# lwy2020/MicroMix

Measured on AMD Instinct MI355X. Metric: mixed-MX GEMM TFLOPS (Llama-3-8B 4096x4096x4096, all-MXFP8 activations, MXFP4 weights), higher is better.
Workload: dtype mxfp8 x mxfp4 -> f32 acc -> bf16; 1 GPU; BASELINE.json configs[1]: 4096^3 mixed-MX GEMM, (p4,p6,p8)=(0,0,4096), w4 weights; M=4096, N=4096, K=4096, parallelism=single GPU

## Files before the change

micromix_amd/csrc/mx_gemm_tile.inc:

```
#define MM_SMALL (MM_WM <= 2)
namespace MM_NS {

__device__ __forceinline__ int mm_tid() { return (int)threadIdx.x; }
constexpr int WM = MM_WM, TM = MM_TM, TN = MM_TN;
constexpr int BM = WM * TM * 32, BN = 2 * TN * 32, NT = WM * 2 * 64;
constexpr bool SMALL = MM_SMALL;
constexpr int NTHREADS = SMALL ? 2 * NT : NT;
constexpr int NACC = 16 * TM * TN;
typedef float v16f_t __attribute__((ext_vector_type(16)));
typedef int v8i_t __attribute__((ext_vector_type(8)));
typedef int v4i_sel __attribute__((ext_vector_type(4)));
struct Acc {
#if MM_SMALL
    v16f_t t[TM * TN];
#endif
};
constexpr int X_TILE = BM * 128;
constexpr int SF_BYTES = 1024;

constexpr int LDS_BUDGET = MM_LDS_BUDGET;

template <int N>
__device__ __forceinline__ void wait_vmcnt() {
#if !(MM_DBG & 2048)
    MM_DEVICE_ONLY(asm volatile("s_waitcnt vmcnt(%0)" ::"n"(N) : "memory");)
#endif
}
__device__ __forceinline__ void barrier_lds_only() {
#if (MM_DBG & 1024)
    MM_DEVICE_ONLY(asm volatile("s_waitcnt lgkmcnt(0)" ::: "memory");)
#else
    MM_DEVICE_ONLY(asm volatile("s_waitcnt lgkmcnt(0)\n\ts_barrier" ::: "memory");)
#endif
}

template <int EL, int KD> struct Op;
template <> struct Op<EL_FP8, 128> { static constexpr int PITCH = 128, G128 = 128; };
template <> struct Op<EL_FP6, 128> { static constexpr int PITCH = 128, G128 = 96; };
template <> struct Op<EL_FP4, 128> { static constexpr int PITCH = 64, G128 = 64; };
template <> struct Op<EL_FP4, 256> { static constexpr int PITCH = 128, G128 = 64; };

template <int EL> struct Frag;
template <> struct Frag<EL_FP8> { typedef int type __attribute__((ext_vector_type(8))); };
template <> struct Frag<EL_FP6> { typedef int type __attribute__((ext_vector_type(6))); };
template <> struct Frag<EL_FP4> { typedef int type __attribute__((ext_vector_type(4))); };

template <int EL, int KD> struct FragOfs;
template <> struct FragOfs<EL_FP8, 128> {
    int o[2][2];
    __device__ __forceinline__ void init(int row, int kb) {
        const int sw = (row >> 1) & 7, rb = row * 128;
#pragma unroll
        for (int h = 0; h < 2; ++h) {
            o[h][0] = rb + (((4 * h + kb) ^ sw) << 4);
            o[h][1] = rb + (((4 * h + 2 + kb) ^ sw) << 4);
        }
    }
};
template <> struct FragOfs<EL_FP4, 128> {
    int o[2][1];
    __device__ __forceinline__ void init(int row, int kb) {
        const int sw = (row >> 2) & 3, rb = row * 64;
#pragma unroll
        for (int h = 0; h < 2; ++h) o[h][0] = rb + (((2 * h + kb) ^ sw) << 4);
    }
};
template <> struct FragOfs<EL_FP4, 256> {
    int o[4][1];
    __device__ __forceinline__ void init(int row, int kb) {
        const int sw = (row >> 1) & 7, rb = row * 128;
#pragma unroll
        for (int h = 0; h < 4; ++h) o[h][0] = rb + (((2 * h + kb) ^ sw) << 4);
    }
};
template <> struct FragOfs<EL_FP6, 128> {
    int o[2][3];
    __device__ __forceinline__ void init(int row, int kb) {
        const int sw = (row >> 1) & 7, rb = row * 128;
#pragma unroll
        for (int h = 0; h < 2; ++h)
#pragma unroll
            for (int i = 0; i < 3; ++i) {
                const int u = 3 * (2 * h + kb) + i;
// ... 38 lines not shown
    const u4_t hi = *(lds_u4)(unsigned long)a1;
    return typename Frag<EL>::type{(int)lo.x, (int)lo.y, (int)lo.z, (int)lo.w, (int)hi.x, (int)hi.y, (int)hi.z, (int)hi.w};
}
template <class G, int EL> using FragOfsOf = std::conditional_t<G::XEL == EL_FP8 && G::WEL == EL_FP8 && !MM_SMALL, FragOfsC<EL, G::KD>, FragOfs<EL, G::KD>>;

template <int T, int XEL, int WEL, int HSEL, bool FENCE = false>
__device__ __forceinline__ void mfma_tile(const typename Frag<XEL>::type &x, const typename Frag<WEL>::type &w, int sx,
                                          int sw) {
#if !(MM_DBG & 1)
    if constexpr (FENCE) {
        MM_DEVICE_ONLY(asm volatile("s_nop 1\n\tv_mfma_scale_f32_32x32x64_f8f6f4 a[%c7:%c8], %0, %1, a[%c7:%c8], %2, %3 "
                                    "op_sel_hi:[%c4,%c4,0] cbsz:%c5 blgp:%c6"
                                    :
                                    : "v"(x), "v"(w), "v"(sx), "v"(sw), "i"(HSEL), "i"(ElemTraits<XEL>::HW),
                                      "i"(ElemTraits<WEL>::HW), "i"(16 * T), "i"(16 * T + 15)
                                    : MM_ACC, "memory");)
    } else {
        MM_DEVICE_ONLY(asm volatile("s_nop 1\n\tv_mfma_scale_f32_32x32x64_f8f6f4 a[%c7:%c8], %0, %1, a[%c7:%c8], %2, %3 "
                                    "op_sel_hi:[%c4,%c4,0] cbsz:%c5 blgp:%c6"
                                    :
                                    : "v"(x), "v"(w), "v"(sx), "v"(sw), "i"(HSEL), "i"(ElemTraits<XEL>::HW),
                                      "i"(ElemTraits<WEL>::HW), "i"(16 * T), "i"(16 * T + 15)
                                    : MM_ACC);)
    }
#else
    MM_DEVICE_ONLY(asm volatile("" ::"v"(x), "v"(w), "v"(sx), "v"(sw));)
#endif
}

template <int I>
__device__ __forceinline__ float acc_read() {
    float v = 0.0f;
    MM_DEVICE_ONLY(asm volatile("v_accvgpr_read_b32 %0, a[%c1]" : "=v"(v) : "i"(I) : MM_ACC);)
    return v;
}
template <int I>
__device__ __forceinline__ void acc_write(float v) {
    MM_DEVICE_ONLY(asm volatile("v_accvgpr_write_b32 a[%c1], %0" : : "v"(v), "i"(I) : MM_ACC);)
}
__device__ __forceinline__ void acc_settle() { MM_DEVICE_ONLY(asm volatile("s_nop 15\n\ts_nop 7" ::: MM_ACC);) }

template <int I, int N>
struct AccLoop {
    static __device__ __forceinline__ void zero() {
        acc_write<I>(0.0f);
        AccLoop<I + 1, N>::zero();
    }
    static __device__ __forceinline__ void round_bf16() {
        static_assert(I % 8 == 0 && N % 8 == 0, "accumulators are rounded eight at a time");
        MM_DEVICE_ONLY(unsigned r0, r1, r2, r3, r4, r5, r6, r7, p0, p1, p2, p3;
                       asm volatile("v_accvgpr_read_b32 %0, a[%c12]\n\tv_accvgpr_read_b32 %1, a[%c13]\n\t"
                                    "v_accvgpr_read_b32 %2, a[%c14]\n\tv_accvgpr_read_b32 %3, a[%c15]\n\t"
                                    "v_accvgpr_read_b32 %4, a[%c16]\n\tv_accvgpr_read_b32 %5, a[%c17]\n\t"
                                    "v_accvgpr_read_b32 %6, a[%c18]\n\tv_accvgpr_read_b32 %7, a[%c19]\n\t"
                                    "v_cvt_pk_bf16_f32 %8, %0, %1\n\tv_cvt_pk_bf16_f32 %9, %2, %3\n\t"
                                    "v_cvt_pk_bf16_f32 %10, %4, %5\n\tv_cvt_pk_bf16_f32 %11, %6, %7\n\t"
                                    "v_lshlrev_b32 %0, 16, %8\n\tv_and_b32 %1, 0xffff0000, %8\n\t"
                                    "v_lshlrev_b32 %2, 16, %9\n\tv_and_b32 %3, 0xffff0000, %9\n\t"
                                    "v_lshlrev_b32 %4, 16, %10\n\tv_and_b32 %5, 0xffff0000, %10\n\t"
                                    "v_lshlrev_b32 %6, 16, %11\n\tv_and_b32 %7, 0xffff0000, %11\n\t"
                                    "v_accvgpr_write_b32 a[%c12], %0\n\tv_accvgpr_write_b32 a[%c13], %1\n\t"
                                    "v_accvgpr_write_b32 a[%c14], %2\n\tv_accvgpr_write_b32 a[%c15], %3\n\t"
                                    "v_accvgpr_write_b32 a[%c16], %4\n\tv_accvgpr_write_b32 a[%c17], %5\n\t"
                                    "v_accvgpr_write_b32 a[%c18], %6\n\tv_accvgpr_write_b32 a[%c19], %7"
                                    : "=&v"(r0), "=&v"(r1), "=&v"(r2), "=&v"(r3), "=&v"(r4), "=&v"(r5), "=&v"(r6), "=&v"(r7),
                                      "=&v"(p0), "=&v"(p1), "=&v"(p2), "=&v"(p3)
                                    : "i"(I), "i"(I + 1), "i"(I + 2), "i"(I + 3), "i"(I + 4), "i"(I + 5), "i"(I + 6), "i"(I + 7)
                                    : MM_ACC);)
        AccLoop<I + 8, N>::round_bf16();
    }
    static __device__ __forceinline__ void store(float *p) {
        static_assert(I % 4 == 0 && N % 4 == 0, "four accumulator registers per store");
        typedef float v4f __attribute__((ext_vector_type(4)));
        [[maybe_unused]] const v4f v = {acc_read<I>(), acc_read<I + 1>(), acc_read<I + 2>(), acc_read<I + 3>()};
        MM_DEVICE_ONLY(asm volatile("global_store_dwordx4 %0, %1, off sc0 sc1\n\ts_nop 1" ::"v"(p + (I / 4) * NT * 4), "v"(v) : "memory");)
        AccLoop<I + 4, N>::store(p);
    }
};
template <int N>
struct AccLoop<N, N> {
    static __device__ __forceinline__ void zero() {}
    static __device__ __forceinline__ void round_bf16() {}
    static __device__ __forceinline__ void store(float *) {}
};

typedef int rsrc_t __attribute__((ext_vector_type(4)));

__device__ __forceinline__ rsrc_t make_rsrc(const uint8_t *base, unsigned bytes) {
    const unsigned long long v = (unsigned long long)base;
    rsrc_t r;
    r[0] = __builtin_amdgcn_readfirstlane((int)(unsigned)v);
    r[1] = __builtin_amdgcn_readfirstlane((int)((unsigned)(v >> 32) & 0xFFFFu));
    r[2] = __builtin_amdgcn_readfirstlane((int)bytes);
    r[3] = 0x00020000;
    return r;
}

__device__ __forceinline__ void dma16(const rsrc_t &rsrc, int voff, int soff, unsigned lds_addr) {
#if (MM_DBG & 2)
    MM_DEVICE_ONLY(asm volatile("" ::"v"(voff), "s"(rsrc), "s"(lds_addr), "s"(soff));)
    return;
#endif
    MM_DEVICE_ONLY(unsigned keep;
                   asm volatile("s_nop 4\n\ts_mov_b32 %0, m0\n\ts_mov_b32 m0, %3\n\ts_nop 0\n\t"
                                "buffer_load_dwordx4 %1, %2, %4 offen lds\n\ts_mov_b32 m0, %0"
                                : "=&s"(keep)
                                : "v"(voff), "s"(rsrc), "s"(lds_addr), "s"(soff)
                                : "memory");)
}

typedef int v4i_t __attribute__((ext_vector_type(4)));
__device__ __forceinline__ __amdgpu_buffer_rsrc_t make_brsrc(const uint8_t *base, unsigned bytes) {
    const unsigned long long v = (unsigned long long)base;
    const unsigned lo = __builtin_amdgcn_readfirstlane((unsigned)v), hi = __builtin_amdgcn_readfirstlane((unsigned)(v >> 32));
    return __builtin_amdgcn_make_buffer_rsrc((void *)(((unsigned long long)hi << 32) | lo), 0,
                                             (int)__builtin_amdgcn_readfirstlane(bytes), 0x00020000);
}
constexpr int OOB = 1 << 30;

__device__ __forceinline__ unsigned lds_address(const uint8_t *p) {
    return (unsigned)(unsigned long long)p;
}

template <int PITCH, int ROWS>
struct OperandDma {
    static constexpr int CPR = PITCH / 16;
    static constexpr int PIECES = ROWS * CPR / NT;
    static_assert(ROWS * CPR % NT == 0, "tile must be a whole number of wave instructions");
    static constexpr int ROWS_PER_IT = NT / CPR;
    rsrc_t rsrc;
    __amdgpu_buffer_rsrc_t brsrc;
    int voff0;
    int rowbytes;
    int g128;
    __device__ __forceinline__ void init(const uint8_t *base, int row0, int nrows, int nslab128, int g128_) {
        g128 = __builtin_amdgcn_readfirstlane(g128_);
        rowbytes = __builtin_amdgcn_readfirstlane(nslab128 * g128);
        int rows = nrows - row0;
        rows = rows > ROWS ? ROWS : rows;
        if constexpr (SMALL) brsrc = make_brsrc(base + (size_t)row0 * (unsigned)rowbytes, (unsigned)rows * (unsigned)rowbytes);
        if constexpr (!SMALL) rsrc = make_rsrc(base + (size_t)row0 * (unsigned)rowbytes, (unsigned)rows * (unsigned)rowbytes);
        const int tid = mm_tid() & (NT - 1);
        const int row = tid / CPR;
        int c;
        if constexpr (CPR == 4) c = (tid & 3) ^ ((row >> 2) & 3);
        else c = (tid & 7) ^ ((row >> 1) & 7);
        if (g128 == 96) c = c >= 6 ? c - 6 : c;
        voff0 = row * rowbytes + c * 16;
    }
    template <int IT>
    __device__ __forceinline__ void piece(int slab128, const uint8_t *lds_tile, int wave) const {
#if (MM_DBG & 16384)
        if constexpr (CPR == 8 && PIECES == 4) {
            const int tid = mm_tid() & (NT - 1);
            const int v = ((IT >> 1) * (NT / 4) + (tid >> 2)) * rowbytes + ((tid & 3) + 4 * (IT & 1)) * 16;
            dma16(rsrc, v, __builtin_amdgcn_readfirstlane(slab128 * g128),
                  __builtin_amdgcn_readfirstlane(lds_address(lds_tile) + (IT * NT + wave * 64) * 16));
            return;
        }
#endif
        dma16(rsrc, voff0 + IT * ROWS_PER_IT * rowbytes, __builtin_amdgcn_readfirstlane(slab128 * g128),
              __builtin_amdgcn_readfirstlane(lds_address(lds_tile) + (IT * NT + wave * 64) * 16));
    }
    template <int IT>
    __device__ __forceinline__ v4i_t load(int slab128, int oob) const {
        return __builtin_amdgcn_raw_buffer_load_b128(brsrc, voff0 + IT * ROWS_PER_IT * rowbytes + oob,
// ... 514 lines not shown
#pragma unroll
                    for (int e = 0; e < 8; ++e)
                        if (n + e < a.N) dst[e] = (uint16_t)(w[e >> 1] >> (16 * (e & 1)));
                }
            }
        }
    }
    template <int GI, int I = 0>
    __device__ __forceinline__ void mfmas_with_rounding() {
        if constexpr (I < 8) {
            mfma<(GI >> 1), (GI & 1), I>();
            if constexpr (GI > 0) round_chunk<((GI - 1) >> 1), ((GI - 1) & 1), I>();
            mfmas_with_rounding<GI, I + 1>();
        }
    }
    template <int GI>
    __device__ __forceinline__ void group() {
        if constexpr (GI < 4) {
            constexpr int TM_ = GI >> 1, P = GI & 1;
            if constexpr (P == 0) load_x<TM_>();
            load_w<2 * P>(ws[0]);
            load_w<2 * P + 1>(ws[1]);
            mfmas_with_rounding<GI>();
        } else {
#if MM_CLOCKS
            if (a.clock_out != nullptr && mm_tid() == 0) {
                a.clock_out[4 * blockIdx.x] = __builtin_amdgcn_s_memtime();
                a.clock_out[4 * blockIdx.x + 1] = __builtin_amdgcn_s_memrealtime();
            }
#endif
            round_chunk<1, 1, 0>(); round_chunk<1, 1, 1>(); round_chunk<1, 1, 2>(); round_chunk<1, 1, 3>();
            round_chunk<1, 1, 4>(); round_chunk<1, 1, 5>(); round_chunk<1, 1, 6>(); round_chunk<1, 1, 7>();
        }
        if constexpr (GI > 0) store_group<((GI - 1) >> 1), ((GI - 1) & 1)>();
        if constexpr (GI < 4) group<GI + 1>();
    }
};

template <class G, class FX, class FW>
__device__ __forceinline__ void run_tail(const GemmArgs &a, int m0, int n0, uint8_t *smem, int c2, int c1, int cf, const Scales<G::KD> &sca,
                                         const FX &fx, const FW &fw, int gx, int gw) {
    const int lane = mm_tid() & 63, wave = __builtin_amdgcn_readfirstlane(mm_tid() >> 6);
    const int wm = wave >> 1, wn = wave & 1, li = lane & 31, kb = lane >> 5;
    wait_vmcnt<0>();
    barrier_lds_only();
    TailTM<G, FX, FW> t{a, smem + c2 * G::STAGE, smem + c1 * G::STAGE, smem + cf * G::STAGE + wave * (32 * TAIL_EP), fx, fw};
    t.sca = sca;
    load_scales<G>(t.scb, t.sb, gx, gw, li, kb);
    t.m0w = m0 + wm * (TM * 32);
    t.n0w = n0 + wn * (TN * 32);
    t.lane = lane;
    t.li = li;
    t.hi = lane >> 5;
    t.sel = (lane & 1) ? 0x03020706u : 0x05040100u;
#pragma unroll
    for (int tn = 0; tn < TN; ++tn) {
        const int n = t.n0w + tn * 32 + li;
        t.bias[tn] = (a.bias != nullptr && n < a.N) ? bf16_bits_to_f32(a.bias[n]) : 0.0f;
    }
    t.template group<0>();
}


template <class G, bool CH, class NX, class PRE, bool TAIL = false>
__device__ __forceinline__ int run_slabs_big(const GemmArgs &a, int Q, int nslab128, int first128, int count, int m0, int n0,
                                             uint8_t *smem, PRE pre, int pref_in, int cur0, const NX &nxd, int nx_pref) {
    constexpr int XEL = G::XEL, WEL = G::WEL, KD = G::KD;
    constexpr bool SAME = CH && (KD == NX::KD), DIFF = CH && (KD != NX::KD);
    static_assert(!TAIL || G::NSTAGE == 3, "the tail runs on a three-stage ring");
    static_assert(!SAME || (NX::STAGE == G::STAGE && NX::NPIECES == SlabDma<G>::NPIECES), "a same-geometry successor continues the ring");
    const int lane = mm_tid() & 63, wave = __builtin_amdgcn_readfirstlane(mm_tid() >> 6);
    const int wm = wave >> 1, wn = wave & 1;
    const int li = lane & 31, kb = lane >> 5;

    SlabDma<G> dma;
    init_slab_dma<G>(dma, a, Q, m0, n0, nslab128, first128, wave);

    constexpr int NS = G::NSTAGE;
    static_assert(NS == 2 || NS == 3, "this pipeline is written out for two or three stages");
    static_assert(!DIFF || NS == 2, "a successor of another geometry needs the two-stage ring (see Chaining above run_slabs_big)");
    auto stage_at = [&](int i) { return smem + i * G::STAGE; };
    auto next_of = [&](int i) { return (i + 1 == NS) ? 0 : i + 1; };
    int cur = cur0;
    const int vcount = count + (SAME ? nx_pref : 0);
    {
        int st = cur;
#pragma unroll
        for (int v = 0; v < NS; ++v) {
            if (v >= pref_in) {
                if (v < count) dma.all(v, stage_at(st));
                else if (SAME && v < vcount) nxd.all(v - count, stage_at(st));
            }
            st = next_of(st);
        }
    }
    if (pref_in == 0) {
        pre();
        if (NS == 3 && vcount > 2) wait_slabs<2>(dma);
        else if (vcount > 1) wait_slabs<1>(dma);
        else wait_slabs<0>(dma);
        barrier_lds_only();
    }

    FragOfsOf<G, XEL> fx;
    FragOfsOf<G, WEL> fw;
    fx.init(wm * (TM * 32) + li, kb);
    fw.init(wn * (TN * 32) + li, kb);
    typename Frag<XEL>::type x0[TM], x1[TM];
    typename Frag<WEL>::type w0[TN], w1[TN];
    Scales<KD> sc;
#pragma unroll
    for (int t = 0; t < TM; ++t) x0[t] = load_frag<XEL, KD, 0>(stage_at(cur), fx, t);
#pragma unroll
    for (int t = 0; t < TN; ++t) w0[t] = load_frag<WEL, KD, 0>(stage_at(cur) + G::OFF_W, fw, t);
    const int gx = ((m0 & 127) >> 5) + wm * TM, gw = ((n0 & 127) >> 5) + wn * TN;
    load_scales<G>(sc, stage_at(cur), gx, gw, li, kb);
    if (pref_in != 0) pre();

#ifdef MM_PRESSURE
    int keep_[MM_PRESSURE];
#pragma unroll
    for (int i = 0; i < MM_PRESSURE; ++i) { keep_[i] = lane * (i + 3); MM_DEVICE_ONLY(asm volatile("" : "+v"(keep_[i]));) }
#endif
    for (int s = 0; s < (TAIL ? count - 2 : count); ++s) {
        const int nxt = next_of(cur);
        uint8_t *st_cur = stage_at(cur);
        uint8_t *st_nxt = stage_at(nxt);
        inner_steps<G, 0>(x0, x1, w0, w1, sc, fx, fw, st_cur);
        if (NS == 3 && s + 2 < vcount) wait_slabs<1>(dma);
        else wait_slabs<0>(dma);
        barrier_lds_only();
        Scales<KD> scn;
        load_scales<G>(scn, st_nxt, gx, gw, li, kb);
        auto lx = [&](auto t) { x0[decltype(t)::value] = load_frag<XEL, KD, 0>(st_nxt, fx, decltype(t)::value); };
        auto lw = [&](auto t) { w0[decltype(t)::value] = load_frag<WEL, KD, 0>(st_nxt + G::OFF_W, fw, decltype(t)::value); };
        constexpr int HL = G::KSTEPS - 1;
        const int v = s + NS;
        if (v < count) {
            mfma_step<XEL, WEL, (HL & 1), SlabPiecesT<SlabDma<G>>>(x1, w1, sc.x[HL >> 1], sc.w[HL >> 1], SlabPiecesT<SlabDma<G>>{dma, v, st_cur}, lx, lw);
        } else if (SAME && v - count < nx_pref) {
            mfma_step<XEL, WEL, (HL & 1), SlabPiecesT<NX>>(x1, w1, sc.x[HL >> 1], sc.w[HL >> 1], SlabPiecesT<NX>{nxd, v - count, st_cur}, lx, lw);
        } else if (DIFF && nx_pref > 0 && v == count) {
            mfma_step<XEL, WEL, (HL & 1), SlabPiecesT<NX>>(x1, w1, sc.x[HL >> 1], sc.w[HL >> 1], SlabPiecesT<NX>{nxd, 0, smem}, lx, lw);
        } else if (DIFF && nx_pref > 1 && v == count + 1) {
            mfma_step<XEL, WEL, (HL & 1), TwoSlabPieces<NX>>(x1, w1, sc.x[HL >> 1], sc.w[HL >> 1], TwoSlabPieces<NX>{nxd, nx_pref, smem}, lx, lw);
        } else {
            mfma_step<XEL, WEL, (HL & 1), NoDma>(x1, w1, sc.x[HL >> 1], sc.w[HL >> 1], NoDma{}, lx, lw);
        }
        sc = scn;
        cur = nxt;
    }
#ifdef MM_PRESSURE
#pragma unroll
    for (int i = 0; i < MM_PRESSURE; ++i) { MM_DEVICE_ONLY(asm volatile("" ::"v"(keep_[i]));) }
#endif
    if constexpr (TAIL) {
        run_tail<G>(a, m0, n0, smem, cur, next_of(cur), next_of(next_of(cur)), sc, fx, fw, gx, gw);
    }
    return cur;
}

template <class G, bool CH, class NX, class PRE, bool TAIL = false>
__device__ __forceinline__ int run_slabs(Acc &acc, const GemmArgs &a, int Q, int nslab128, int first128, int count, int m0, int n0,
                                         uint8_t *smem, PRE pre, int pref_in, int cur0, const NX &nxd, int nx_pref) {
    if constexpr (SMALL) {
        static_assert(!TAIL, "the tail belongs to the 8-wave pipeline");
        run_slabs_small<G>(acc, a, Q, nslab128, first128, count, m0, n0, smem, pre);
        return 0;
    } else {
        return run_slabs_big<G, CH, NX, PRE, TAIL>(a, Q, nslab128, first128, count, m0, n0, smem, pre, pref_in, cur0, nxd, nx_pref);
    }
}

template <bool W4> struct Segs {
    using N256 = Geom<EL_FP4, EL_FP4, 256>;
    using N128 = Geom<EL_FP4, EL_FP4, 128>;
    using S = Geom<EL_FP6, (W4 ? EL_FP4 : EL_FP6), 128>;
    using O = Geom<EL_FP8, (W4 ? EL_FP4 : EL_FP8), 128>;
    using DmaSO = SlabDma<S>;
    static_assert(std::is_same<SlabDma<S>, SlabDma<O>>::value && S::NSTAGE == O::NSTAGE, "S and O chain through one ring");
    static constexpr bool CHAIN = (MM_CHAIN && W4 && BM == 256 && !SMALL && MM_FP4_KD256 && N256::NSTAGE == 2 && S::STAGE <= N256::STAGE &&
                                   S::NSTAGE * S::STAGE <= LDS_BUDGET);
    static constexpr int EPILOGUE = (NT / 64) * 32 * 320 + ((WM == 4 && TN == 4) ? 1024 + (NT / 64) * 2048 : 0);
    static constexpr int cmax(int x, int y) { return x > y ? x : y; }
    static constexpr int TOTAL = cmax(cmax(cmax(N256::BYTES, N128::BYTES), cmax(S::BYTES, O::BYTES)), EPILOGUE);
    static_assert(TOTAL <= LDS_BUDGET, "LDS budget");
};
template <bool W4> struct Lds { static constexpr int TOTAL = Segs<W4>::TOTAL; };

template <bool W4, int Q, class PRE>
__device__ __forceinline__ void run_segment(Acc &acc, const GemmArgs &a, int nslab128, int first, int count, int m0, int n0, uint8_t *smem,
                                            PRE pre) {
    using SG = Segs<W4>;
    const typename SG::DmaSO none{};
    if constexpr (Q == 0) {
#if MM_FP4_KD256 && MM_WM >= 2
        const int n2 = count >> 1;
        if (n2) run_slabs<typename SG::N256, false>(acc, a, 0, nslab128, first, n2, m0, n0, smem, pre, 0, 0, none, 0);
        if (count & 1) {
            if (n2) {
                barrier_lds_only();
                run_slabs<typename SG::N128, false>(acc, a, 0, nslab128, first + 2 * n2, 1, m0, n0, smem, [] {}, 0, 0, none, 0);
            } else {
                run_slabs<typename SG::N128, false>(acc, a, 0, nslab128, first, 1, m0, n0, smem, pre, 0, 0, none, 0);
            }
        }
#else
        run_slabs<typename SG::N128, false>(acc, a, 0, nslab128, first, count, m0, n0, smem, pre, 0, 0, none, 0);
#endif
    } else if constexpr (Q == 1) {
        run_slabs<typename SG::S, false>(acc, a, 1, nslab128, first, count, m0, n0, smem, pre, 0, 0, none, 0);
    } else {
        run_slabs<typename SG::O, false>(acc, a, 2, nslab128, first, count, m0, n0, smem, pre, 0, 0, none, 0);
    }
}

template <bool W4, bool TAIL, class RND>
__device__ __forceinline__ void run_all_segments(Acc &acc, const GemmArgs &a, int n0s, int n1s, int n2s, int m0, int n0, uint8_t *smem,
                                                 RND round_acc) {
    using SG = Segs<W4>;
    using DmaSO = typename SG::DmaSO;
    static_assert(!TAIL || SG::CHAIN, "the tail is built into the chained segment sequence of the 256-row tile");
    auto nothing = [] {};
    if constexpr (!SG::CHAIN) {
        if (n0s) run_segment<W4, 0>(acc, a, n0s, 0, n0s, m0, n0, smem, nothing);
        if (n1s) {
            if (n0s) {
                barrier_lds_only();
                run_segment<W4, 1>(acc, a, n1s, 0, n1s, m0, n0, smem, round_acc);
            } else {
                run_segment<W4, 1>(acc, a, n1s, 0, n1s, m0, n0, smem, nothing);
            }
        }
        if (n2s) {
            if (n0s | n1s) {
                barrier_lds_only();
                run_segment<W4, 2>(acc, a, n2s, 0, n2s, m0, n0, smem, round_acc);
            } else {
                run_segment<W4, 2>(acc, a, n2s, 0, n2s, m0, n0, smem, nothing);
            }
        }
    } else {
        const int wave = __builtin_amdgcn_readfirstlane(mm_tid() >> 6);
        constexpr int NSO = SG::S::NSTAGE;
        const int qn = n1s ? 1 : 2, cn = n1s ? n1s : n2s;
        const bool chain_n = n0s >= 4 && !(n0s & 1) && cn > 0;
        DmaSO dn, d2;
        dn.init(a, qn, m0, n0, cn, 0, wave, n1s ? Op<SG::S::XEL, 128>::G128 : Op<SG::O::XEL, 128>::G128,
                n1s ? Op<SG::S::WEL, 128>::G128 : Op<SG::O::WEL, 128>::G128);
        const bool chain_s = n1s > 0 && n2s > 0;
        d2.init(a, 2, m0, n0, n2s, 0, wave, Op<SG::O::XEL, 128>::G128, Op<SG::O::WEL, 128>::G128);
        int pref = 0, cur = 0;
        bool any = false;
        auto pre = [&] {
            if (any) round_acc();
        };
        if (n0s) {
            if (chain_n) {
                const int n2 = n0s >> 1;
                pref = cn < NSO ? cn : NSO;
                run_slabs<typename SG::N256, true>(acc, a, 0, n0s, 0, n2, m0, n0, smem, nothing, 0, n2 & 1, dn, pref);
            } else {
                run_segment<W4, 0>(acc, a, n0s, 0, n0s, m0, n0, smem, nothing);
            }
            any = true;
        }
        if (n1s) {
            if (any && pref == 0) barrier_lds_only();
            const int pout = chain_s ? (n2s < NSO ? n2s : NSO) : 0;
            cur = run_slabs<typename SG::S, true>(acc, a, 1, n1s, 0, n1s, m0, n0, smem, pre, pref, 0, d2, pout);
            pref = pout;
            any = true;
        }
        if (n2s) {
            if (any && pref == 0) barrier_lds_only();
            run_slabs<typename SG::O, true, DmaSO, decltype(pre), TAIL>(acc, a, 2, n2s, 0, n2s, m0, n0, smem, pre, pref, pref ? cur : 0, d2, 0);
        }
    }
}

#ifndef MM_PP_CPIECES
#define MM_PP_CPIECES 0
#endif
#ifndef MM_PP_FLIP
#define MM_PP_FLIP 0
#endif
template <class G>
struct PingPong {
    using D = SlabDma<G>;
    static constexpr int XEL = G::XEL, WEL = G::WEL, KD = G::KD, CP = MM_PP_CPIECES;
    static_assert(G::KSTEPS == 2 && G::NSTAGE == 3 && TM == 2 && TN == 4, "the ping-pong loop is written for the 256 x 256 tile on a three-stage 128-deep ring");
    static_assert(D::SFW <= 4, "the scale pieces are issued by waves of G0 only (G1's vmcnt counts none)");
    static_assert(CP >= 0 && CP <= 2 && CP < D::XP, "compute-phase pieces are activation pieces");
    using XF = typename Frag<XEL>::type;
    using WF = typename Frag<WEL>::type;
    const D &dma;
    const FragOfsOf<G, XEL> &fx;
    const FragOfsOf<G, WEL> &fw;
    int gx, gw, li, kb;
    XF x[2][TM];
    WF w[2][TN];
    Scales<KD> sc;

    template <int H>
    __device__ __forceinline__ void read_step(const uint8_t *st) {
#pragma unroll
        for (int t = 0; t < TM; ++t) x[H][t] = load_frag<XEL, KD, H>(st, fx, t);
#pragma unroll
        for (int t = 0; t < TN; ++t) w[H][t] = load_frag<WEL, KD, H>(st + G::OFF_W, fw, t);
    }
    template <int P = CP>
    __device__ __forceinline__ void mem_pieces(int slab, uint8_t *stage) const {
        if constexpr (P < D::NPIECES) {
            dma.template piece<P>(slab, stage);
            mem_pieces<P + 1>(slab, stage);
        }
    }
    __device__ __forceinline__ void memory(const uint8_t *st, int ahead, uint8_t *st_ahead) {
        read_step<0>(st);
        read_step<1>(st);
        load_scales<G>(sc, st, gx, gw, li, kb);
        mem_pieces(ahead, st_ahead);
        MM_DEVICE_ONLY(asm volatile("" : "+v"(sc.x[0][0]), "+v"(sc.x[0][1]), "+v"(sc.w[0][0]), "+v"(sc.w[0][1]), "+v"(sc.w[0][2]),
                                    "+v"(sc.w[0][3]));)
    }
    template <int I = 0>
    __device__ __forceinline__ void compute(int ahead, uint8_t *st_ahead) const {
        if constexpr (I < 16) {
            constexpr int H = I >> 3, P = I & 7, tn = P / TM, tm = P % TM;
            mfma_tile<tn * TM + tm, XEL, WEL, H>(x[H][tm], w[H][tn], sc.x[0][tm], sc.w[0][tn]);
            if constexpr ((I & 1) && (I >> 1) < CP) dma.template piece<(I >> 1)>(ahead, st_ahead);
            compute<I + 1>(ahead, st_ahead);
        }
    }
};

template <class G>
__device__ __forceinline__ void run_pingpong(const GemmArgs &a, int count, int m0, int n0, uint8_t *smem) {
    using D = SlabDma<G>;
    const int lane = mm_tid() & 63, wave = __builtin_amdgcn_readfirstlane(mm_tid() >> 6);
    const int wm = wave >> 1, wn = wave & 1, li = lane & 31, kb = lane >> 5;
    const bool g1 = wave >= NT / 128;
    D dma;
    init_slab_dma<G>(dma, a, 2, m0, n0, count, 0, wave);
    auto stage_at = [&](int i) { return smem + i * G::STAGE; };
    dma.all(0, stage_at(0));
    dma.all(1, stage_at(1));
    wait_slabs<1>(dma);
    barrier_lds_only();
    FragOfsOf<G, G::XEL> fx;
    FragOfsOf<G, G::WEL> fw;
    fx.init(wm * (TM * 32) + li, kb);
    fw.init(wn * (TN * 32) + li, kb);
    const int gx = ((m0 & 127) >> 5) + wm * TM, gw = ((n0 & 127) >> 5) + wn * TN;
    PingPong<G> pp{dma, fx, fw, gx, gw, li, kb};
#if MM_PP_FLIP && MM_PRIO
    MM_DEVICE_ONLY(asm volatile("s_setprio 0");)
#endif
    const int P = count - 2;
    if (g1 && P > 0) barrier_lds_only();
    int st = 0;
    for (int s = 0; s < P; ++s) {
        const int sa = st == 0 ? 2 : st - 1;
        pp.memory(stage_at(st), s + 2, stage_at(sa));
        if (g1) wait_vmcnt<D::NPIECES - 1 - PingPong<G>::CP>();
        barrier_lds_only();
#if MM_PP_FLIP
        MM_DEVICE_ONLY(asm volatile("s_setprio 1");)
#endif
        pp.compute(s + 2, stage_at(sa));
#if MM_PP_FLIP
        MM_DEVICE_ONLY(asm volatile("s_setprio 0");)
#endif
        if (!g1) wait_slabs<1>(dma);
        MM_DEVICE_ONLY(__builtin_amdgcn_sched_barrier(0);)
        barrier_lds_only();
        st = st == 2 ? 0 : st + 1;
    }
    if (!g1 && P > 0) barrier_lds_only();
    const int c1 = st == 2 ? 0 : st + 1, cf = c1 == 2 ? 0 : c1 + 1;
    Scales<G::KD> sca;
    load_scales<G>(sca, stage_at(st), gx, gw, li, kb);
    run_tail<G>(a, m0, n0, smem, st, c1, cf, sca, fx, fw, gx, gw);
}

__device__ __forceinline__ void write_tile(const GemmArgs &a, Acc &acc, const int m0, const int n0, uint8_t *smem) {
    const int lane = mm_tid() & 63, wave = mm_tid() >> 6;
    const int wm = wave >> 1, wn = wave & 1;
    const int li = lane & 31, hi = lane >> 5;
#if MM_SMALL
#define MM_ACC_GET(T_, I_) acc.t[T_][I_]
#else
#define MM_ACC_GET(T_, I_) acc_read<16 * (T_) + (I_)>()
#endif
    if (a.out_f32) {
        float *D32 = reinterpret_cast<float *>(a.D);
#define MM_F32_TILE(TM_, TN_)                                                                              \
        {                                                                                                  \
            float v[16];                                                                                   \
            v[0] = MM_ACC_GET(TN_ * TM + TM_, 0);   v[1] = MM_ACC_GET(TN_ * TM + TM_, 1);                  \
            v[2] = MM_ACC_GET(TN_ * TM + TM_, 2);   v[3] = MM_ACC_GET(TN_ * TM + TM_, 3);                  \
            v[4] = MM_ACC_GET(TN_ * TM + TM_, 4);   v[5] = MM_ACC_GET(TN_ * TM + TM_, 5);                  \
            v[6] = MM_ACC_GET(TN_ * TM + TM_, 6);   v[7] = MM_ACC_GET(TN_ * TM + TM_, 7);                  \
            v[8] = MM_ACC_GET(TN_ * TM + TM_, 8);   v[9] = MM_ACC_GET(TN_ * TM + TM_, 9);                  \
            v[10] = MM_ACC_GET(TN_ * TM + TM_, 10); v[11] = MM_ACC_GET(TN_ * TM + TM_, 11);                \
            v[12] = MM_ACC_GET(TN_ * TM + TM_, 12); v[13] = MM_ACC_GET(TN_ * TM + TM_, 13);                \
            v[14] = MM_ACC_GET(TN_ * TM + TM_, 14); v[15] = MM_ACC_GET(TN_ * TM + TM_, 15);                \
            const int n = n0 + wn * (TN * 32) + TN_ * 32 + li;                                             \
            _Pragma("unroll") for (int r = 0; r < 16; ++r) {                                               \
                           \
                const int m = m0 + wm * (TM * 32) + TM_ * 32 + 8 * (r >> 2) + 4 * hi + (r & 3);            \
                if (n < a.N && m < a.M) D32[(size_t)m * a.N + n] = v[r];                                   \
            }                                                                                              \
        }
#if MM_TN == 4
#define MM_F32_ROW(TM_) MM_F32_TILE(TM_, 0) MM_F32_TILE(TM_, 1) MM_F32_TILE(TM_, 2) MM_F32_TILE(TM_, 3)
#elif MM_TN == 2
#define MM_F32_ROW(TM_) MM_F32_TILE(TM_, 0) MM_F32_TILE(TM_, 1)
#else
#define MM_F32_ROW(TM_) MM_F32_TILE(TM_, 0)
#endif
        MM_F32_ROW(0)
#if MM_TM >= 2
        MM_F32_ROW(1)
#endif
#if MM_TM == 4
        MM_F32_ROW(2)
        MM_F32_ROW(3)
#endif
#undef MM_F32_ROW
#undef MM_F32_TILE
        return;
    }
    constexpr int EP = 320;
    uint8_t *reg = smem + wave * (32 * EP);
    float bias[TN];
#pragma unroll
    for (int tn = 0; tn < TN; ++tn) {
        const int n = n0 + wn * (TN * 32) + tn * 32 + li;
        bias[tn] = (a.bias != nullptr && n < a.N) ? bf16_bits_to_f32(a.bias[n]) : 0.0f;
    }
    const bool vec_ok = (a.N & 7) == 0;
    [[maybe_unused]] const unsigned sel = (lane & 1) ? 0x03020706u : 0x05040100u;
    uint8_t *wr = reg + (4 * hi + (lane & 1)) * EP + (li & ~1) * 2;
    const int rgrp = ((0x96 >> ((lane >> 2) & 7)) & 1) + 2 * hi, ridx = ((lane >> 3) & 3) * 4 + (lane & 3);
    auto store_rows = [&](int tm) {
        constexpr int RPI = 16 / TN;
#pragma unroll
        for (int j = 0; j < 32 / RPI; ++j) {
// ... 335 lines not shown
#pragma unroll
        for (int i = 0; i < 16; ++i) run[t][i] = sum[t][i] = 0.0f;
    auto fold = [&] {
#pragma unroll
        for (int t = 0; t < NF; ++t)
#pragma unroll
            for (int i = 0; i < 16; i += 2) {
                const float t0 = sum[t][i] + run[t][i], t1 = sum[t][i + 1] + run[t][i + 1];
                sum[t][i] = sum[t][i + 1] = 0.0f;
                if (a.round_per_segment) {
                    unsigned pk = 0;
                    MM_DEVICE_ONLY(asm("v_cvt_pk_bf16_f32 %0, %1, %2" : "=v"(pk) : "v"(t0), "v"(t1));)
                    run[t][i] = __uint_as_float(pk << 16);
                    run[t][i + 1] = __uint_as_float(pk & 0xFFFF0000u);
                } else {
                    run[t][i] = t0;
                    run[t][i + 1] = t1;
                }
            }
    };
    int cur_seg = (int)(a.slot_seg & 3ull);
    for (int sb = 0; sb < nslots; sb += B) {
        v4i_t v[B][CHUNKS];
#pragma unroll
        for (int b = 0; b < B; ++b)
            if (sb + b < nslots) {
                const int soff = __builtin_amdgcn_readfirstlane((sb + b) * PART_BYTES);
#pragma unroll
                for (int c = 0; c < CHUNKS; ++c) v[b][c] = __builtin_amdgcn_raw_buffer_load_b128(rs, tofs + c * (NT * 16), soff, AUX_SC);
            }
#pragma unroll
        for (int b = 0; b < B; ++b)
            if (sb + b < nslots) {
                const int sg = (int)((a.slot_seg >> (2 * (sb + b))) & 3ull);
                if (sg != cur_seg) {
                    fold();
                    cur_seg = sg;
                }
#pragma unroll
                for (int c = 0; c < CHUNKS; ++c)
#pragma unroll
                    for (int e = 0; e < 4; ++e) sum[c >> 2][4 * (c & 3) + e] += __int_as_float(v[b][c][e]);
            }
    }
    fold();
#pragma unroll
    for (int t = 0; t < NF; ++t)
#pragma unroll
        for (int i = 0; i < 16; ++i) acc.t[t][i] = run[t][i];
#if MM_CLOCKS
    if (ck != nullptr && mm_tid() == 0) ck[4] = __builtin_amdgcn_s_memrealtime() - r0;
#endif
    write_tile(a, acc, m0, n0, smem);
#if MM_CLOCKS
    if (ck != nullptr && mm_tid() == 0) {
        asm volatile("s_waitcnt vmcnt(0)" ::: "memory");
        ck[5] = __builtin_amdgcn_s_memrealtime() - r0;
    }
#endif
#endif
}

template <bool W4, bool SPLITK, bool ACT = false, bool TAIL = false, bool PP = false, bool BF16H = false>
__device__ __forceinline__ void tile_body(const GemmArgs &a, const int bid) {
    static_assert(!TAIL || (!SPLITK && !ACT), "the tail replaces the plain bf16 epilogue only");
    static_assert(!PP || (W4 && TAIL), "the ping-pong loop hands over to the tile-major tail");
    extern __shared__ __attribute__((aligned(128))) uint8_t smem[];
    Acc acc;

    const int tiles_m = (a.M + BM - 1) / BM, tiles_n = a.n_tiles ? a.n_tiles : (a.N + BN - 1) / BN;
    const int n0s = a.K[0] >> 7, n1s = a.K[1] >> 7, n2s = a.K[2] >> 7;
    if constexpr (SPLITK && SMALL) {
        split_tile_reduce<W4>(a, bid, acc, smem);
        return;
    } else if constexpr (SPLITK) {
        const int q = bid % a.splits, tile = bid / a.splits;
        const int m0 = __builtin_amdgcn_readfirstlane((tile / tiles_n) * BM);
        const int n0 = __builtin_amdgcn_readfirstlane((tile % tiles_n) * BN);
        const int seg = (q >= a.split_first[1]) + (q >= a.split_first[2]);
        const int j = q - a.split_first[seg], parts = a.split_first[seg + 1] - a.split_first[seg];
        const int ns = a.K[seg] >> 7;
        const int first = __builtin_amdgcn_readfirstlane(ns * j / parts);
        const int count = __builtin_amdgcn_readfirstlane(ns * (j + 1) / parts - first);
        AccLoop<0, NACC>::zero();
        if (seg == 0) run_segment<W4, 0>(acc, a, ns, first, count, m0, n0, smem, [] {});
        else if (seg == 1) run_segment<W4, 1>(acc, a, ns, first, count, m0, n0, smem, [] {});
        else run_segment<W4, 2>(acc, a, ns, first, count, m0, n0, smem, [] {});
        acc_settle();
        AccLoop<0, NACC>::store(a.ws + (size_t)bid * (NACC * NT) + 4 * mm_tid());
        return;
    }

#if MM_PRIO && MM_WM == 4
    if (__builtin_amdgcn_readfirstlane(mm_tid()) >= 256) { MM_DEVICE_ONLY(asm volatile("s_setprio %0" ::"n"(MM_PRIO));) }
#endif
    const int ntiles = tiles_m * tiles_n;
    auto map_tile = [&](int id, int &m0_, int &n0_) {
        {
            const int q = ntiles >> 3, r = ntiles & 7, xcd = id & 7, j = id >> 3;
            id = (xcd < r ? xcd * (q + 1) : r * (q + 1) + (xcd - r) * q) + j;
        }
#ifdef MM_GH
        constexpr int GH = MM_GH;
#else
        constexpr int GH = 4;
#endif
        const int per_group = GH * tiles_n;
        const int grp = id / per_group;
        const int first_m = grp * GH;
        const int gh = (tiles_m - first_m) < GH ? (tiles_m - first_m) : GH;
        const int in = id - grp * per_group;
        m0_ = __builtin_amdgcn_readfirstlane((first_m + in % gh) * BM);
        n0_ = __builtin_amdgcn_readfirstlane((a.n_tile0 + in / gh) * BN);
    };
    auto round_acc = [&] {
        if (a.round_per_segment) {
#if MM_SMALL
#pragma unroll
            for (int t = 0; t < TM * TN; ++t)
#pragma unroll
                for (int i = 0; i < 16; i += 2) {
                    unsigned pk = 0;
                    MM_DEVICE_ONLY(asm("v_cvt_pk_bf16_f32 %0, %1, %2" : "=v"(pk) : "v"(acc.t[t][i]), "v"(acc.t[t][i + 1]));)
                    acc.t[t][i] = __uint_as_float(pk << 16);
                    acc.t[t][i + 1] = __uint_as_float(pk & 0xFFFF0000u);
                }
#else
            acc_settle();
            AccLoop<0, NACC>::round_bf16();
#endif
        }
    };
    {
        int m0, n0;
        map_tile(bid, m0, n0);
#if MM_CLOCKS
        unsigned long long t0 = 0, r0 = 0;
        const bool stamp = a.clock_out != nullptr;
        if (stamp) {
            t0 = __builtin_amdgcn_s_memtime();
            r0 = __builtin_amdgcn_s_memrealtime();
        }
#endif
#if MM_SMALL
#pragma unroll
        for (int t = 0; t < TM * TN; ++t)
#pragma unroll
            for (int i = 0; i < 16; ++i) acc.t[t][i] = 0.0f;
#else
        AccLoop<0, NACC>::zero();
#endif
#if (MM_DBG & 4096)
        const int lm0 = 0, ln0 = 0;
#elif (MM_DBG & 8192)
        const int lm0 = __builtin_amdgcn_readfirstlane((bid & 7) * BM), ln0 = __builtin_amdgcn_readfirstlane((bid & 7) * BN);
#else
        const int lm0 = m0, ln0 = n0;
#endif
        if constexpr (PP) run_pingpong<typename Segs<W4>::O>(a, n2s, lm0, ln0, smem);
        else run_all_segments<W4, TAIL>(acc, a, n0s, n1s, n2s, lm0, ln0, smem, round_acc);
        if constexpr (TAIL) {
#if MM_CLOCKS
            if (stamp && mm_tid() == 0) {
                a.clock_out[4 * bid] -= t0;
                a.clock_out[4 * bid + 1] -= r0;
                a.clock_out[4 * bid + 2] = r0;
                asm volatile("s_waitcnt vmcnt(0)" ::: "memory");
                a.clock_out[4 * bid + 3] = __builtin_amdgcn_s_memrealtime() - r0;
            }
#endif
            return;
        }
        __syncthreads();
        if constexpr (SMALL) {
            if (mm_tid() >= NT) return;
        } else {
            acc_settle();
        }
#if MM_CLOCKS
        if (stamp && mm_tid() == 0) {
            a.clock_out[4 * bid] = __builtin_amdgcn_s_memtime() - t0;
            a.clock_out[4 * bid + 1] = __builtin_amdgcn_s_memrealtime() - r0;
            a.clock_out[4 * bid + 2] = r0;
        }
#endif
#if MM_WM == 4 && MM_TN == 4
        if constexpr (ACT) write_tile_act<BF16H>(a, m0, n0, smem);
        else
#endif
            write_tile(a, acc, m0, n0, smem);
#if MM_CLOCKS
        if (stamp && mm_tid() == 0) {
            asm volatile("s_waitcnt vmcnt(0)" ::: "memory");
            a.clock_out[4 * bid + 3] = __builtin_amdgcn_s_memrealtime() - r0;
        }
#endif
    }
}

template <bool W4, bool SPLITK>
__global__ void __launch_bounds__(NTHREADS) mx_gemm256_kernel(GemmArgs a) {
    tile_body<W4, SPLITK>(a, blockIdx.x);
}
#if MM_WM == 4 && MM_TM == 2
template <bool W4, bool SPLITK, bool TAIL>
__global__ void __launch_bounds__(NTHREADS) mx_gemm256_kernel(GemmArgs a) {
    static_assert(W4 && !SPLITK && TAIL, "the tail kernel exists for fp4 weights without split-K");
    tile_body<W4, SPLITK, false, TAIL>(a, blockIdx.x);
}
template <bool W4, bool SPLITK, bool TAIL, bool PP>
__global__ void __launch_bounds__(NTHREADS) mx_gemm256_kernel(GemmArgs a) {
    static_assert(W4 && !SPLITK && TAIL && PP, "the ping-pong kernel exists for fp4 weights without split-K, with the tail");
    tile_body<W4, SPLITK, false, TAIL, PP>(a, blockIdx.x);
}
#endif
#if MM_WM == 4 && MM_TN == 4
__global__ void __launch_bounds__(NTHREADS) mx_gemm256_act_kernel(GemmArgs a) {
    tile_body<true, false, true>(a, blockIdx.x);
}
#endif

template <bool W4>
__global__ void __launch_bounds__(NTHREADS) mx_gemm256_grouped_kernel(GroupedTileArgs ga) {
    int g = 0;
#pragma unroll
    for (int i = 1; i < MM_MAX_GROUPS; ++i) g += (i < ga.ngroups && (int)blockIdx.x >= ga.first_block[i]) ? 1 : 0;
    tile_body<W4, false>(ga.g[g], (int)blockIdx.x - ga.first_block[g]);
}

template <bool W4>
__global__ void __launch_bounds__(NTHREADS) mx_gemm256_moe_kernel(GemmArgs a, MoeGroups mg) {
    const int tiles_n = (a.N + BN - 1) / BN;
    int bid = blockIdx.x, e = 0, lo = 0, M = 0;
    for (; e < mg.E; ++e) {
        lo = mg.offsets[e];
        M = mg.offsets[e + 1] - lo;
        const int t = (lo >= 0 && M > 64 && M <= mg.max_rows && M <= mg.n - lo) ? ((M + BM - 1) / BM) * tiles_n : 0;
        if (bid < t) break;
        bid -= t;
    }
    if (e >= mg.E) return;
    moe_group_args(a, mg, e, lo, M);
    tile_body<W4, false>(a, bid);
// ... 22 lines not shown
```

micromix_amd/csrc/mx_instrument.h:

```cpp
#pragma once
#ifdef MM_INSTRUMENT
#ifndef MM_DBG
#define MM_DBG 0
#endif
#define MM_CLOCKS 1
#else
#ifdef MM_DBG
#error "MM_DBG ablation switches need -DMM_INSTRUMENT (tools/build_variant.sh)"
#endif
#define MM_DBG 0
#define MM_CLOCKS 0
#endif
```

Before: 2959 TFLOP/s.

## Overlap accumulator zeroing and first-slab setup with head DMA in GEMM prologue

```diff
diff --git a/micromix_amd/csrc/mx_gemm_tile.inc b/micromix_amd/csrc/mx_gemm_tile.inc
--- a/micromix_amd/csrc/mx_gemm_tile.inc
+++ b/micromix_amd/csrc/mx_gemm_tile.inc
@@ -1,4 +1,10 @@
 #define MM_SMALL (MM_WM <= 2)
+#ifndef MM_HEAD_EARLY_DMA
+#define MM_HEAD_EARLY_DMA 1
+#endif
+#ifndef MM_HEAD_SLAB0_FIRST
+#define MM_HEAD_SLAB0_FIRST 1
+#endif
 namespace MM_NS {
 
 __device__ __forceinline__ int mm_tid() { return (int)threadIdx.x; }
@@ -203,6 +209,12 @@
     static __device__ __forceinline__ void zero() {}
     static __device__ __forceinline__ void round_bf16() {}
     static __device__ __forceinline__ void store(float *) {}
+};
+struct ZeroAcc {
+    static constexpr bool LIGHT = true;
+    __device__ __forceinline__ void operator()() const {
+        if constexpr (MM_HEAD_EARLY_DMA) AccLoop<0, NACC>::zero();
+    }
 };
 
 typedef int rsrc_t __attribute__((ext_vector_type(4)));
@@ -883,6 +895,7 @@
     auto stage_at = [&](int i) { return smem + i * G::STAGE; };
     auto next_of = [&](int i) { return (i + 1 == NS) ? 0 : i + 1; };
     int cur = cur0;
+    constexpr bool LIGHT = MM_HEAD_SLAB0_FIRST && requires { PRE::LIGHT; };
     const int vcount = count + (SAME ? nx_pref : 0);
     {
         int st = cur;
@@ -892,11 +905,14 @@
                 if (v < count) dma.all(v, stage_at(st));
                 else if (SAME && v < vcount) nxd.all(v - count, stage_at(st));
             }
+            if constexpr (LIGHT) {
+                if (v == 0 && pref_in == 0) pre();
+            }
             st = next_of(st);
         }
     }
     if (pref_in == 0) {
-        pre();
+        if constexpr (!LIGHT) pre();
         if (NS == 3 && vcount > 2) wait_slabs<2>(dma);
         else if (vcount > 1) wait_slabs<1>(dma);
         else wait_slabs<0>(dma);
@@ -1016,21 +1032,20 @@
     }
 }
 
-template <bool W4, bool TAIL, class RND>
+template <bool W4, bool TAIL, class RND, class FIRST>
 __device__ __forceinline__ void run_all_segments(Acc &acc, const GemmArgs &a, int n0s, int n1s, int n2s, int m0, int n0, uint8_t *smem,
-                                                 RND round_acc) {
+                                                 RND round_acc, FIRST first) {
     using SG = Segs<W4>;
     using DmaSO = typename SG::DmaSO;
     static_assert(!TAIL || SG::CHAIN, "the tail is built into the chained segment sequence of the 256-row tile");
-    auto nothing = [] {};
     if constexpr (!SG::CHAIN) {
-        if (n0s) run_segment<W4, 0>(acc, a, n0s, 0, n0s, m0, n0, smem, nothing);
+        if (n0s) run_segment<W4, 0>(acc, a, n0s, 0, n0s, m0, n0, smem, first);
         if (n1s) {
             if (n0s) {
                 barrier_lds_only();
                 run_segment<W4, 1>(acc, a, n1s, 0, n1s, m0, n0, smem, round_acc);
             } else {
-                run_segment<W4, 1>(acc, a, n1s, 0, n1s, m0, n0, smem, nothing);
+                run_segment<W4, 1>(acc, a, n1s, 0, n1s, m0, n0, smem, first);
             }
         }
         if (n2s) {
@@ -1038,7 +1053,7 @@
                 barrier_lds_only();
                 run_segment<W4, 2>(acc, a, n2s, 0, n2s, m0, n0, smem, round_acc);
             } else {
-                run_segment<W4, 2>(acc, a, n2s, 0, n2s, m0, n0, smem, nothing);
+                run_segment<W4, 2>(acc, a, n2s, 0, n2s, m0, n0, smem, first);
             }
         }
     } else {
@@ -1055,14 +1070,15 @@
         bool any = false;
         auto pre = [&] {
             if (any) round_acc();
+            else first();
         };
         if (n0s) {
             if (chain_n) {
                 const int n2 = n0s >> 1;
                 pref = cn < NSO ? cn : NSO;
-                run_slabs<typename SG::N256, true>(acc, a, 0, n0s, 0, n2, m0, n0, smem, nothing, 0, n2 & 1, dn, pref);
+                run_slabs<typename SG::N256, true>(acc, a, 0, n0s, 0, n2, m0, n0, smem, first, 0, n2 & 1, dn, pref);
             } else {
-                run_segment<W4, 0>(acc, a, n0s, 0, n0s, m0, n0, smem, nothing);
+                run_segment<W4, 0>(acc, a, n0s, 0, n0s, m0, n0, smem, first);
             }
             any = true;
         }
@@ -1117,11 +1133,11 @@
             mem_pieces<P + 1>(slab, stage);
         }
     }
-    __device__ __forceinline__ void memory(const uint8_t *st, int ahead, uint8_t *st_ahead) {
+    __device__ __forceinline__ void memory(const uint8_t *st, int ahead, uint8_t *st_ahead, bool pieces = true) {
         read_step<0>(st);
         read_step<1>(st);
         load_scales<G>(sc, st, gx, gw, li, kb);
-        mem_pieces(ahead, st_ahead);
+        if (pieces) mem_pieces(ahead, st_ahead);
         MM_DEVICE_ONLY(asm volatile("" : "+v"(sc.x[0][0]), "+v"(sc.x[0][1]), "+v"(sc.w[0][0]), "+v"(sc.w[0][1]), "+v"(sc.w[0][2]),
                                     "+v"(sc.w[0][3]));)
     }
@@ -1136,8 +1152,16 @@
     }
 };
 
-template <class G>
-__device__ __forceinline__ void run_pingpong(const GemmArgs &a, int count, int m0, int n0, uint8_t *smem) {
+#ifndef MM_PP_HEAD
+#define MM_PP_HEAD 2
+#endif
+struct HeadClock {
+    unsigned long long t0, r0;
+    int bid;
+};
+template <class G, class PRE>
+__device__ __forceinline__ void run_pingpong(const GemmArgs &a, int count, int m0, int n0, uint8_t *smem, PRE pre,
+                                             [[maybe_unused]] const HeadClock &hc) {
     using D = SlabDma<G>;
     const int lane = mm_tid() & 63, wave = __builtin_amdgcn_readfirstlane(mm_tid() >> 6);
     const int wm = wave >> 1, wn = wave & 1, li = lane & 31, kb = lane >> 5;
@@ -1146,26 +1170,71 @@
     init_slab_dma<G>(dma, a, 2, m0, n0, count, 0, wave);
     auto stage_at = [&](int i) { return smem + i * G::STAGE; };
     dma.all(0, stage_at(0));
+#if MM_PP_HEAD != 2
     dma.all(1, stage_at(1));
-    wait_slabs<1>(dma);
-    barrier_lds_only();
+#endif
+    pre();
     FragOfsOf<G, G::XEL> fx;
     FragOfsOf<G, G::WEL> fw;
     fx.init(wm * (TM * 32) + li, kb);
     fw.init(wn * (TN * 32) + li, kb);
     const int gx = ((m0 & 127) >> 5) + wm * TM, gw = ((n0 & 127) >> 5) + wn * TN;
+#if MM_PP_HEAD == 2
+    MM_DEVICE_ONLY(asm volatile("" : "+v"(fx.o[0][0]), "+v"(fw.o[0][0]));)
+    dma.all(1, stage_at(1));
+#endif
     PingPong<G> pp{dma, fx, fw, gx, gw, li, kb};
+    wait_slabs<1>(dma);
+    barrier_lds_only();
 #if MM_PP_FLIP && MM_PRIO
     MM_DEVICE_ONLY(asm volatile("s_setprio 0");)
+#endif
+#if MM_CLOCKS
+    auto stamp_first = [&] {
+        if (a.clock_out != nullptr && (mm_tid() & 255) == 0 && hc.bid < MM_CLOCK_WGS) {
+            unsigned long long *p = a.clock_out + MM_CLOCK_HEAD + 4 * hc.bid + (g1 ? 2 : 0);
+            p[0] = __builtin_amdgcn_s_memtime() - hc.t0;
+            p[1] = __builtin_amdgcn_s_memrealtime() - hc.r0;
+        }
+    };
+#else
+    auto stamp_first = [] {};
 #endif
     const int P = count - 2;
     if (g1 && P > 0) barrier_lds_only();
     int st = 0;
-    for (int s = 0; s < P; ++s) {
+    int s = 0;
+#if MM_PP_HEAD
+    if (P > 0) {
+        pp.memory(stage_at(0), 2, stage_at(2), g1);
+        if (g1) wait_vmcnt<D::NPIECES - 1 - PingPong<G>::CP>();
+        barrier_lds_only();
+        stamp_first();
+#if MM_PP_FLIP
+        MM_DEVICE_ONLY(asm volatile("s_setprio 1");)
+#endif
+        pp.compute(2, stage_at(2));
+#if MM_PP_FLIP
+        MM_DEVICE_ONLY(asm volatile("s_setprio 0");)
+#endif
+        if (!g1) {
+            pp.mem_pieces(2, stage_at(2));
+            wait_slabs<1>(dma);
+        }
+        MM_DEVICE_ONLY(__builtin_amdgcn_sched_barrier(0);)
+        barrier_lds_only();
+        st = 1;
+        s = 1;
+    }
+#endif
+    for (; s < P; ++s) {
         const int sa = st == 0 ? 2 : st - 1;
         pp.memory(stage_at(st), s + 2, stage_at(sa));
         if (g1) wait_vmcnt<D::NPIECES - 1 - PingPong<G>::CP>();
         barrier_lds_only();
+#if !MM_PP_HEAD
+        if (s == 0) stamp_first();
+#endif
 #if MM_PP_FLIP
         MM_DEVICE_ONLY(asm volatile("s_setprio 1");)
 #endif
@@ -1667,10 +1736,11 @@
         const int ns = a.K[seg] >> 7;
         const int first = __builtin_amdgcn_readfirstlane(ns * j / parts);
         const int count = __builtin_amdgcn_readfirstlane(ns * (j + 1) / parts - first);
-        AccLoop<0, NACC>::zero();
-        if (seg == 0) run_segment<W4, 0>(acc, a, ns, first, count, m0, n0, smem, [] {});
-        else if (seg == 1) run_segment<W4, 1>(acc, a, ns, first, count, m0, n0, smem, [] {});
-        else run_segment<W4, 2>(acc, a, ns, first, count, m0, n0, smem, [] {});
+        const ZeroAcc zero_acc;
+        if constexpr (!MM_HEAD_EARLY_DMA) AccLoop<0, NACC>::zero();
+        if (seg == 0) run_segment<W4, 0>(acc, a, ns, first, count, m0, n0, smem, zero_acc);
+        else if (seg == 1) run_segment<W4, 1>(acc, a, ns, first, count, m0, n0, smem, zero_acc);
+        else run_segment<W4, 2>(acc, a, ns, first, count, m0, n0, smem, zero_acc);
         acc_settle();
         AccLoop<0, NACC>::store(a.ws + (size_t)bid * (NACC * NT) + 4 * mm_tid());
         return;
@@ -1732,8 +1802,10 @@
         for (int t = 0; t < TM * TN; ++t)
 #pragma unroll
             for (int i = 0; i < 16; ++i) acc.t[t][i] = 0.0f;
+        auto zero_acc = [] {};
 #else
-        AccLoop<0, NACC>::zero();
+        if constexpr (!MM_HEAD_EARLY_DMA) AccLoop<0, NACC>::zero();
+        const ZeroAcc zero_acc;
 #endif
 #if (MM_DBG & 4096)
         const int lm0 = 0, ln0 = 0;
@@ -1742,8 +1814,13 @@
 #else
         const int lm0 = m0, ln0 = n0;
 #endif
-        if constexpr (PP) run_pingpong<typename Segs<W4>::O>(a, n2s, lm0, ln0, smem);
-        else run_all_segments<W4, TAIL>(acc, a, n0s, n1s, n2s, lm0, ln0, smem, round_acc);
+#if MM_CLOCKS
+        const HeadClock hc{t0, r0, bid};
+#else
+        const HeadClock hc{0, 0, bid};
+#endif
+        if constexpr (PP) run_pingpong<typename Segs<W4>::O>(a, n2s, lm0, ln0, smem, zero_acc, hc);
+        else run_all_segments<W4, TAIL>(acc, a, n0s, n1s, n2s, lm0, ln0, smem, round_acc, zero_acc);
         if constexpr (TAIL) {
 #if MM_CLOCKS
             if (stamp && mm_tid() == 0) {
diff --git a/micromix_amd/csrc/mx_instrument.h b/micromix_amd/csrc/mx_instrument.h
--- a/micromix_amd/csrc/mx_instrument.h
+++ b/micromix_amd/csrc/mx_instrument.h
@@ -4,6 +4,8 @@
 #define MM_DBG 0
 #endif
 #define MM_CLOCKS 1
+#define MM_CLOCK_WGS 4096
+#define MM_CLOCK_HEAD (4 * MM_CLOCK_WGS)
 #else
 #ifdef MM_DBG
 #error "MM_DBG ablation switches need -DMM_INSTRUMENT (tools/build_variant.sh)"
```

Result: no change. 2980 TFLOP/s, median of 5 (+0.7%).
